# Twilight-Dream-Of-Magic/KolmogorovLike-DataCompressor

Measured on AMD Instinct MI355X. Metric: compress MB/s at fixed block size, bit-exact vs reference; 1/2/4/8-GPU scaling, higher is better.
Workload: dtype u8; 1 GPU; enwik-style synthetic text (kolm.datagen.enwik_like, seed 20251212+rank), 256 MiB per GPU resident in HBM, 1 MiB fixed blocks, candidates 0..8 + MDL, payloads emitted in HBM; block_size=1048576, bytes_per_gpu=268435456, blocks_per_gpu=256, parallelism=block-shard x1

## Files before the change

### kolmogorovlike-datacompressor_amd/csrc/k_mtf.hip

```cpp
#include "kolm_internal.h"

namespace kolm {

namespace {

struct ChunkGeom {
    Geom geo;
    u32 cpb;
    u32 csz;
    __device__ inline bool range(u32 c, u32& lo, u32& hi) const {
        const u32 b = c / cpb;
        const u32 k = c - b * cpb;
        lo = geo.base(b) + k * csz;
        const u32 e = geo.end(b);
        hi = min(lo + csz, e);
        return lo < e;
    }
};

constexpr u32 MTF_SLAB = 64;

__global__ __launch_bounds__(256) void k_mtf_summary(ChunkGeom cg, const u8* in, u8* summary,
                                                     u16* scnt, u32 nchunks) {
    __shared__ u32 sl[256 * MTF_SLAB / 4];
    __shared__ u32 slo[256];
    const u32 t = threadIdx.x;
    const u32 c = blockIdx.x * blockDim.x + t;
    u32 lo = 0, hi = 0;
    const bool valid = c < nchunks && cg.range(c, lo, hi);
    u16 cnt = 0;
    if (__syncthreads_and(valid && hi - lo == cg.csz && (lo & 15) == 0)) {
        u32 seen[8] = {0, 0, 0, 0, 0, 0, 0, 0};
        u8* out = summary + (u64)c * 256;
        slo[t] = lo;
        __syncthreads();
        for (u32 r = cg.csz; r > 0; r -= MTF_SLAB) {
#pragma unroll
            for (u32 q = 0; q < MTF_SLAB / 16; ++q) {
                const u32 m = q * 256 + t, owner = m >> 2, part = m & 3;
                reinterpret_cast<uint4*>(sl)[m] =
                    *reinterpret_cast<const uint4*>(in + slo[owner] + r - MTF_SLAB + 16 * part);
            }
            __syncthreads();
            const u32* slab = sl + t * (MTF_SLAB / 4);
#pragma unroll
            for (int q = MTF_SLAB / 4 - 1; q >= 0; --q) {
                const u32 wv = slab[q];
#pragma unroll
                for (int j = 3; j >= 0; --j) {
                    const u32 b = (wv >> (8 * j)) & 0xFF, w = b >> 5, bit = 1u << (b & 31);
                    u32 sw = 0;
#pragma unroll
                    for (int k = 0; k < 8; ++k) sw = (k == (int)w) ? seen[k] : sw;
                    if (!(sw & bit)) {
#pragma unroll
                        for (int k = 0; k < 8; ++k)
                            if (k == (int)w) seen[k] |= bit;
                        out[cnt++] = (u8)b;
                    }
                }
            }
            __syncthreads();
        }
        scnt[c] = cnt;
        return;
    }
    if (!valid) {
        if (c < nchunks) scnt[c] = 0;
        return;
    }
    {
        u32 seen[8] = {0, 0, 0, 0, 0, 0, 0, 0};
        u8* out = summary + (u64)c * 256;
        auto visit = [&](u32 b) {
            const u32 w = b >> 5, bit = 1u << (b & 31);
            u32 sw = 0;
#pragma unroll
            for (int k = 0; k < 8; ++k) sw = (k == (int)w) ? seen[k] : sw;
            if (!(sw & bit)) {
#pragma unroll
                for (int k = 0; k < 8; ++k)
                    if (k == (int)w) seen[k] |= bit;
                out[cnt++] = (u8)b;
            }
        };
        if (((lo | hi) & 15) == 0) {
            for (u32 i = hi; i > lo; i -= 16) {
                const uint4 v = *reinterpret_cast<const uint4*>(in + i - 16);
                const u32 wv[4] = {v.x, v.y, v.z, v.w};
#pragma unroll
                for (int q = 3; q >= 0; --q)
#pragma unroll
                    for (int j = 3; j >= 0; --j) visit((wv[q] >> (8 * j)) & 0xFF);
            }
        } else {
            for (u32 i = hi; i > lo; --i) visit(in[i - 1]);
        }
    }
    scnt[c] = cnt;
}

__device__ inline void mtf_apply(u32* st, u8* nst, u32* member, const u8* sm, u32 cnt) {
    const u32 lane = threadIdx.x & 63;
    if (lane < 8) member[lane] = 0;
    __builtin_amdgcn_wave_barrier();
    __builtin_amdgcn_fence(__ATOMIC_RELEASE, "wavefront");
    u32 sv[4];
#pragma unroll
    for (int j = 0; j < 4; ++j) {
        const u32 i = 4 * lane + j;
        sv[j] = i < cnt ? sm[i] : 0;
        if (i < cnt) atomicOr(&member[sv[j] >> 5], 1u << (sv[j] & 31));
    }
    __builtin_amdgcn_fence(__ATOMIC_ACQ_REL, "wavefront");
    __builtin_amdgcn_wave_barrier();
    const u32 word = st[lane];
    u32 keep = 0;
    u8 e[4];
#pragma unroll
    for (int j = 0; j < 4; ++j) {
        e[j] = (word >> (8 * j)) & 0xFF;
        const bool in_sum = (member[e[j] >> 5] >> (e[j] & 31)) & 1u;
        keep |= (in_sum ? 0u : 1u) << j;
    }
    const u32 nk = __popc(keep);
    u32 pos = cnt + wave_incl_scan(nk, OpAddU(), 0u) - nk;
#pragma unroll
    for (int j = 0; j < 4; ++j) {
        const u32 i = 4 * lane + j;
        if (i < cnt) nst[i] = (u8)sv[j];
        if ((keep >> j) & 1u) nst[pos++] = e[j];
    }
    __builtin_amdgcn_fence(__ATOMIC_ACQ_REL, "wavefront");
    __builtin_amdgcn_wave_barrier();
    st[lane] = reinterpret_cast<const u32*>(nst)[lane];
    __builtin_amdgcn_fence(__ATOMIC_ACQ_REL, "wavefront");
    __builtin_amdgcn_wave_barrier();
}


constexpr u32 CP_W = 16;
constexpr u32 CP_G = 8;
constexpr u32 CP_S = 16;
constexpr u32 CP_R = CP_G * CP_S;

__device__ inline u32 mtf_ident(u32 lane) {
    return (4 * lane) | ((4 * lane + 1) << 8) | ((4 * lane + 2) << 16) | ((4 * lane + 3) << 24);
}

__device__ inline void cp_range(const ChunkGeom& cg, u32 b, u32 r, u32& k0, u32& k1) {
    const u32 nch = (cg.geo.end(b) - cg.geo.base(b) + cg.csz - 1) / cg.csz;
    const u32 per = (nch + CP_R - 1) / CP_R;
    k0 = min(r * per, nch);
    k1 = min(k0 + per, nch);
}

__global__ __launch_bounds__(64 * CP_W) void k_mtf_cp1(ChunkGeom cg, const u8* summary, const u16* scnt, u32* rst,
                                                      u32* rdist) {
    __shared__ u32 st[CP_W][64];
    __shared__ u8 nst[CP_W][256];
    __shared__ u32 member[CP_W][8];
    __shared__ u32 uni[CP_W][8];
    const u32 lane = threadIdx.x & 63, w = threadIdx.x >> 6;
    const u32 gr = blockIdx.x * CP_W + w, b = gr / CP_R, r = gr - b * CP_R;
    if (b >= cg.geo.nb) return;
    u32 k0, k1;
    cp_range(cg, b, r, k0, k1);
    st[w][lane] = mtf_ident(lane);
    if (lane < 8) uni[w][lane] = 0;
    __builtin_amdgcn_wave_barrier();
    for (u32 k = k0; k < k1; ++k) {
        const u32 c = b * cg.cpb + k;
        const u8* sm = summary + (u64)c * 256;
        const u32 cnt = scnt[c];
#pragma unroll
        for (int j = 0; j < 4; ++j) {
            const u32 i = 4 * lane + j;
            if (i < cnt) atomicOr(&uni[w][sm[i] >> 5], 1u << (sm[i] & 31));
        }
        mtf_apply(st[w], nst[w], member[w], sm, cnt);
    }
    __builtin_amdgcn_fence(__ATOMIC_ACQ_REL, "wavefront");
    __builtin_amdgcn_wave_barrier();
    rst[(u64)gr * 64 + lane] = st[w][lane];
    if (lane == 0) {
        u32 d = 0;
        for (int q = 0; q < 8; ++q) d += __popc(uni[w][q]);
        rdist[gr] = d;
    }
}

__global__ __launch_bounds__(64 * CP_G) void k_mtf_cp2(const u32* rst, const u32* rdist, u32* rentry) {
    __shared__ u32 st[CP_G][64];
    __shared__ u8 nst[CP_G][256];
    __shared__ u32 member[CP_G][8];
    __shared__ u32 uni[CP_G][8];
    __shared__ u8 gsum[CP_G][256];
    __shared__ u32 gentry[CP_G][64];
    __shared__ u32 gdist[CP_G];
    const u32 lane = threadIdx.x & 63, g = threadIdx.x >> 6, b = blockIdx.x;
    const u64 r0 = (u64)b * CP_R + g * CP_S;
    st[g][lane] = mtf_ident(lane);
    if (lane < 8) uni[g][lane] = 0;
    __builtin_amdgcn_wave_barrier();
    for (u32 v = 0; v < CP_S; ++v) {
        const u8* sm = reinterpret_cast<const u8*>(rst + (r0 + v) * 64);
        const u32 cnt = rdist[r0 + v];
#pragma unroll
        for (int j = 0; j < 4; ++j) {
            const u32 i = 4 * lane + j;
            if (i < cnt) atomicOr(&uni[g][sm[i] >> 5], 1u << (sm[i] & 31));
        }
        mtf_apply(st[g], nst[g], member[g], sm, cnt);
    }
    __builtin_amdgcn_fence(__ATOMIC_ACQ_REL, "wavefront");
    __builtin_amdgcn_wave_barrier();
    reinterpret_cast<u32*>(gsum[g])[lane] = st[g][lane];
    if (lane == 0) {
        u32 d = 0;
        for (int q = 0; q < 8; ++q) d += __popc(uni[g][q]);
        gdist[g] = d;
    }
    __syncthreads();
    if (g == 0) {
        st[0][lane] = mtf_ident(lane);
        __builtin_amdgcn_wave_barrier();
        for (u32 v = 0; v < CP_G; ++v) {
            gentry[v][lane] = st[0][lane];
            __builtin_amdgcn_fence(__ATOMIC_ACQ_REL, "wavefront");
            __builtin_amdgcn_wave_barrier();
            if (v + 1 < CP_G) mtf_apply(st[0], nst[0], member[0], gsum[v], gdist[v]);
        }
    }
    __syncthreads();
    st[g][lane] = gentry[g][lane];
    __builtin_amdgcn_wave_barrier();
    for (u32 v = 0; v < CP_S; ++v) {
        rentry[(r0 + v) * 64 + lane] = st[g][lane];
        mtf_apply(st[g], nst[g], member[g], reinterpret_cast<const u8*>(rst + (r0 + v) * 64), rdist[r0 + v]);
    }
}

__global__ __launch_bounds__(64 * CP_W) void k_mtf_cp3(ChunkGeom cg, const u8* summary, const u16* scnt,
                                                      const u32* rentry, u8* states) {
    __shared__ u32 st[CP_W][64];
    __shared__ u8 nst[CP_W][256];
    __shared__ u32 member[CP_W][8];
    const u32 lane = threadIdx.x & 63, w = threadIdx.x >> 6;
    const u32 gr = blockIdx.x * CP_W + w, b = gr / CP_R, r = gr - b * CP_R;
    if (b >= cg.geo.nb) return;
    u32 k0, k1;
    cp_range(cg, b, r, k0, k1);
    st[w][lane] = rentry[(u64)gr * 64 + lane];
    __builtin_amdgcn_wave_barrier();
    for (u32 k = k0; k < k1; ++k) {
        const u32 c = b * cg.cpb + k;
        reinterpret_cast<u32*>(states + (u64)c * 256)[lane] = st[w][lane];
        mtf_apply(st[w], nst[w], member[w], summary + (u64)c * 256, scnt[c]);
    }
}

constexpr int RT = 128;

struct RiceAcc {
    u32 c[5] = {0, 0, 0, 0, 0};
    int k;
    u32 kk = 0, km = 0;
    __device__ inline void init(int rk) {
        k = rk;
        kk = rk < 8 ? (u32)rk : 0u;
        km = rk < 8 ? (0xFFu >> rk) * 0x01010101u : 0u;
    }
    __device__ inline u32 rb(u32 v) const { return (v >> k) + 1 + k; }
    __device__ inline u32 sum4(u32 w, u32 a) const { return __builtin_amdgcn_sad_u8((w >> kk) & km, 0u, a); }
    __device__ inline void add(u32 v) {
        c[0] += rb(v);
        c[2] += rb(((v & 0x0Fu) << 4) | (v >> 4));
        c[3] += rb(__brev(v) >> 24);
        c[4] += rb(v ^ (v >> 1));
    }
    __device__ inline void add4(u32 o) {
        const u32 one = 4 * (1 + k);
        c[0] = sum4(o, c[0] + one);
        c[2] = sum4(((o & 0x0F0F0F0Fu) << 4) | ((o >> 4) & 0x0F0F0F0Fu), c[2] + one);
        c[3] = sum4(__brev(o), c[3] + one);
        c[4] = sum4(o ^ ((o >> 1) & 0x7F7F7F7Fu), c[4] + one);
    }
    __device__ inline void group(u32 lo, u32 hi) {
        u64 x = ((u64)__builtin_bswap32(lo) << 32) | __builtin_bswap32(hi);
        u64 t = (x ^ (x >> 7)) & 0x00AA00AA00AA00AAull;
        x ^= t ^ (t << 7);
        t = (x ^ (x >> 14)) & 0x0000CCCC0000CCCCull;
        x ^= t ^ (t << 14);
        t = (x ^ (x >> 28)) & 0x00000000F0F0F0F0ull;
        x ^= t ^ (t << 28);
        c[1] = sum4((u32)(x >> 32), sum4((u32)x, c[1] + 8 * (1 + k)));
    }
};

__global__ __launch_bounds__(RT) void k_mtf_replay(ChunkGeom cg, const u8* in, const u8* states, u8* out,
                                                   u32 nchunks, u64* bits, int rice_k) {
    __shared__ u32 tab[64 * RT];
    const u32 t = threadIdx.x;
    const u32 c = blockIdx.x * RT + t;
    u32 lo = 0, hi = 0;
    const bool valid = c < nchunks && cg.range(c, lo, hi);
    u32 r0 = 0, r1 = 0;
    if (valid) {
        const u32* s = reinterpret_cast<const u32*>(states + (u64)c * 256);
        r0 = s[0];
        r1 = s[1];
        for (int w = 2; w < 64; ++w) tab[w * RT + t] = s[w];
    }
    auto haszero = [](u32 y) { return (y - 0x01010101u) & ~y & 0x80808080u; };
    auto front = [](u32 x, u32 j, u32 in) {
        const u32 lowmask = j ? ((1u << (8 * j)) - 1) : 0u;
        const u32 highmask = j == 3 ? 0u : ~((1u << (8 * (j + 1))) - 1);
        return (x & highmask) | ((x & lowmask) << 8) | in;
    };
    auto step = [&](u32 b) -> u32 {
        const u32 bb = b * 0x01010101u;
        u32 z = haszero(r0 ^ bb);
        if (z) {
            const u32 j = (__ffs(z) - 1) >> 3;
            r0 = front(r0, j, b);
            return j;
        }
        const u32 c0 = r0 >> 24;
        z = haszero(r1 ^ bb);
        if (z) {
            const u32 j = (__ffs(z) - 1) >> 3;
            r0 = (r0 << 8) | b;
            r1 = front(r1, j, c0);
            return 4 + j;
        }
        u32 w = 2, x;
        for (;;) {
            x = tab[w * RT + t];
            z = haszero(x ^ bb);
            if (z) break;
            ++w;
        }
        const u32 j = (__ffs(z) - 1) >> 3;
        u32 carry = r1 >> 24;
        r1 = (r1 << 8) | c0;
        r0 = (r0 << 8) | b;
        for (u32 v = 2; v < w; ++v) {
            const u32 xv = tab[v * RT + t];
            tab[v * RT + t] = (xv << 8) | carry;
            carry = xv >> 24;
        }
        tab[w * RT + t] = front(x, j, carry);
        return 4 * w + j;
    };
    RiceAcc acc;
    acc.init(rice_k);
    if (!valid) return;
    if (((lo | hi) & 63) == 0) {
        for (u32 i = lo; i < hi; i += 64) {
            uint4 v[4];
#pragma unroll
            for (int h = 0; h < 4; ++h) v[h] = *reinterpret_cast<const uint4*>(in + i + 16 * h);
            u32 ov[16];
#pragma unroll
            for (int q = 0; q < 16; ++q) {
                const u32 wq = q % 4 == 0 ? v[q / 4].x : q % 4 == 1 ? v[q / 4].y : q % 4 == 2 ? v[q / 4].z : v[q / 4].w;
                u32 o = 0;
#pragma unroll
                for (int j = 0; j < 4; ++j) o |= step((wq >> (8 * j)) & 0xFF) << (8 * j);
                ov[q] = o;
                if (bits) acc.add4(o);
                if (bits && (q & 1)) acc.group(ov[q - 1], o);
            }
#pragma unroll
            for (int h = 0; h < 4; ++h)
                *reinterpret_cast<uint4*>(out + i + 16 * h) = make_uint4(ov[4 * h], ov[4 * h + 1], ov[4 * h + 2], ov[4 * h + 3]);
        }
    } else if (((lo | hi) & 15) == 0) {
        for (u32 i = lo; i < hi; i += 16) {
            const uint4 v = *reinterpret_cast<const uint4*>(in + i);
            const u32 wv[4] = {v.x, v.y, v.z, v.w};
            u32 ov[4];
#pragma unroll
            for (int q = 0; q < 4; ++q) {
                u32 o = 0;
#pragma unroll
                for (int j = 0; j < 4; ++j) o |= step((wv[q] >> (8 * j)) & 0xFF) << (8 * j);
                ov[q] = o;
                if (bits) acc.add4(o);
            }
            *reinterpret_cast<uint4*>(out + i) = make_uint4(ov[0], ov[1], ov[2], ov[3]);
            if (bits) {
                acc.group(ov[0], ov[1]);
                acc.group(ov[2], ov[3]);
            }
        }
    } else {
        u32 g[2] = {0, 0}, gi = 0;
        for (u32 i = lo; i < hi; ++i) {
            const u32 m = step(in[i]);
            out[i] = (u8)m;
            if (bits) {
                acc.add(m);
                g[gi >> 2] |= m << (8 * (gi & 3));
                if (++gi == 8) {
                    acc.group(g[0], g[1]);
                    g[0] = g[1] = 0;
                    gi = 0;
                }
            }
        }
        if (bits && gi) acc.group(g[0], g[1]);
    }
    if (bits) {
        u64* dst = bits + (u64)(c / cg.cpb) * 8;
#pragma unroll
        for (int q = 0; q < 5; ++q)
            if (acc.c[q]) atomicAdd((unsigned long long*)&dst[q], (unsigned long long)acc.c[q]);
    }
}

__global__ __launch_bounds__(256) void k_mtf_wave(ChunkGeom cg, const u8* in, const u8* states, u8* out,
                                                  u32 nchunks, u64* bits, int rice_k) {
    __shared__ u32 st[4][64];
    __shared__ u8 nst[4][256];
    __shared__ u32 member[4][8];
    __shared__ u8 inv[4][256];
    __shared__ u8 smy[4][64];
    __shared__ __align__(8) u8 mb[4][64];
    const u32 w = threadIdx.x >> 6, lane = threadIdx.x & 63;
    const u32 c = blockIdx.x * 4 + w;
    u32 lo = 0, hi = 0;
    if (!(c < nchunks && cg.range(c, lo, hi))) return;
    {
        const u32 word = reinterpret_cast<const u32*>(states + (u64)c * 256)[lane];
        st[w][lane] = word;
#pragma unroll
        for (int j = 0; j < 4; ++j) inv[w][(word >> (8 * j)) & 0xFF] = (u8)(4 * lane + j);
    }
    __builtin_amdgcn_fence(__ATOMIC_ACQ_REL, "wavefront");
    __builtin_amdgcn_wave_barrier();
    RiceAcc acc;
    acc.init(rice_k);
    const u64 below = (1ull << lane) - 1ull;
    for (u32 p = lo; p < hi; p += 64) {
        const u32 i = p + lane;
        const bool v = i < hi;
        const u32 sym = v ? in[i] : 0u;
        const u64 vm = __ballot(v);
        const u32 mypos = inv[w][sym];
        u64 rem = vm, mine = 0;
        while (rem) {
            const u32 k = (u32)__ffsll((long long)rem) - 1;
            const u32 sk = __builtin_amdgcn_readlane(sym, k);
            const u64 eq = __ballot(v && sym == sk);
            if (sym == sk) mine = eq;
            rem &= ~eq;
        }
        const u64 pm = mine & below;
        const u32 prev = pm ? 63u - (u32)__clzll((long long)pm) : 0u;
        const u64 win = pm ? below & ~((2ull << prev) - 1ull) : 0ull;
        u32 cnt = 0, seen = 0, less = 0;
        rem = vm;
        while (rem) {
            const u32 k = (u32)__ffsll((long long)rem) - 1;
            const u32 sk = __builtin_amdgcn_readlane(sym, k);
            const u32 pk = __builtin_amdgcn_readlane(mypos, k);
            const u64 eq = __ballot(v && sym == sk);
            cnt += (eq & win) ? 1u : 0u;
            if (k < lane) {
                ++seen;
                less += pk < mypos ? 1u : 0u;
            }
            rem &= ~eq;
        }
        const u32 m = pm ? cnt : seen + mypos - less;
        if (v) out[i] = (u8)m;
        mb[w][lane] = v ? (u8)m : (u8)0;
        if (bits && v) acc.add(m);
        const bool last = v && (mine >> lane) == 1ull;
        const u64 lm = __ballot(last);
        if (last) smy[w][__popcll(lm >> lane) - 1] = (u8)sym;
        __builtin_amdgcn_fence(__ATOMIC_ACQ_REL, "wavefront");
        __builtin_amdgcn_wave_barrier();
        if (bits && (lane & 7) == 0 && v) {
            const u32* g = reinterpret_cast<const u32*>(&mb[w][lane]);
            acc.group(g[0], g[1]);
        }
        mtf_apply(st[w], nst[w], member[w], smy[w], (u32)__popcll(lm));
        const u32 word = st[w][lane];
#pragma unroll
        for (int j = 0; j < 4; ++j) inv[w][(word >> (8 * j)) & 0xFF] = (u8)(4 * lane + j);
        __builtin_amdgcn_fence(__ATOMIC_ACQ_REL, "wavefront");
        __builtin_amdgcn_wave_barrier();
    }
    if (bits) {
        u64* dst = bits + (u64)(c / cg.cpb) * 8;
#pragma unroll
        for (int q = 0; q < 5; ++q) {
            const u32 sum = wave_reduce(acc.c[q], OpAddU(), 0u);
            if (lane == 0 && sum) atomicAdd((unsigned long long*)&dst[q], (unsigned long long)sum);
        }
    }
}

}

bool mtf_wave_mode(const Geom& geo) {
    const char* e = getenv("KOLM_MTF_WAVE");
    const int force = e ? atoi(e) : -1;
    return force >= 0 ? force != 0 : geo.nb < 64;
}

u32 mtf_chunk_bytes(const Geom& geo) {
    static const u32 force = getenv("KOLM_MTF_CHUNK") ? (u32)atoi(getenv("KOLM_MTF_CHUNK")) : 0u;
    if (force >= 64 && force <= MTF_CHUNK && (force & (force - 1)) == 0) return force;
    u32 csz = MTF_CHUNK;
    if (mtf_wave_mode(geo)) return csz;
    while (csz > 128 && (u64)((geo.bs + csz - 1) / csz) * geo.nb < 16384) csz >>= 1;
    return csz;
}

u64 mtf_cp_words(const Geom& geo) { return (u64)geo.nb * CP_R * 129; }

void launch_mtf(const Geom& geo, const u8* in, u8* out, u8* summary, u16* summary_cnt, u8* states,
                hipStream_t s, KTimer* kt, u64* bits, int rice_k, u32* cp_scratch) {
    if (!geo.N) return;
    const u32 csz = mtf_chunk_bytes(geo);
    ChunkGeom cg{geo, (geo.bs + csz - 1) / csz, csz};
    const u32 nchunks = cg.cpb * geo.nb;
    const u64 N = geo.N;
    {
        KScope k(kt, KT_MTF, "k_mtf_summary", N + (u64)nchunks * 256);
        k_mtf_summary<<<(nchunks + 255) / 256, 256, 0, s>>>(cg, in, summary, summary_cnt, nchunks);
    }
    {
        KScope k(kt, KT_MTF, "k_mtf_compose", (u64)nchunks * 512);
        {
            u32* rst = cp_scratch;
            u32* rentry = cp_scratch + (u64)geo.nb * CP_R * 64;
            u32* rdist = rentry + (u64)geo.nb * CP_R * 64;
            const u32 g13 = (geo.nb * CP_R + CP_W - 1) / CP_W;
            k_mtf_cp1<<<g13, 64 * CP_W, 0, s>>>(cg, summary, summary_cnt, rst, rdist);
            k_mtf_cp2<<<geo.nb, 64 * CP_G, 0, s>>>(rst, rdist, rentry);
            k_mtf_cp3<<<g13, 64 * CP_W, 0, s>>>(cg, summary, summary_cnt, rentry, states);
        }
    }
    if (mtf_wave_mode(geo)) {
        KScope k(kt, KT_MTF, "k_mtf_wave", 2 * N + (u64)nchunks * 256);
        k_mtf_wave<<<(nchunks + 3) / 4, 256, 0, s>>>(cg, in, states, out, nchunks, bits, rice_k);
    } else {
        KScope k(kt, KT_MTF, "k_mtf_replay", 2 * N + (u64)nchunks * 256);
        k_mtf_replay<<<(nchunks + RT - 1) / RT, RT, 0, s>>>(cg, in, states, out, nchunks, bits, rice_k);
    }
}

}
```

Before: 8803 MB/s.

## Replace serial MTF range composition with last-occurrence key ranking

The per-range MTF state kernel previously applied each chunk summary sequentially with mtf_apply and atomic union bitmaps. It now records a last-seen key per symbol (chunk index and position stamp) in one pass over the summaries, four chunks at a time, then builds the final MTF order by ranking keys with a 64x4 comparison sweep. This replaces a long serial chain of wave-synchronised list updates with independent scatter writes plus one O(256^2) rank, and shrinks workgroups to 4 waves. It adds a 2^24-chunk limit check and relies on the key ordering reproducing MTF semantics exactly.

```diff
diff --git a/kolmogorovlike-datacompressor_amd/csrc/k_mtf.hip b/kolmogorovlike-datacompressor_amd/csrc/k_mtf.hip
--- a/kolmogorovlike-datacompressor_amd/csrc/k_mtf.hip
+++ b/kolmogorovlike-datacompressor_amd/csrc/k_mtf.hip
@@ -1,4 +1,5 @@
 #include "kolm_internal.h"
+#include "mtf_core.h"
 
 namespace kolm {
 
@@ -139,10 +140,13 @@
 }
 
 
-constexpr u32 CP_W = 16;
-constexpr u32 CP_G = 8;
-constexpr u32 CP_S = 16;
-constexpr u32 CP_R = CP_G * CP_S;
+constexpr u32 CP_W = 4;
+constexpr u32 RS_W = 4;
+constexpr u32 RS_B = 4;
+constexpr u32 CP_G = mtf::GROUPS;
+constexpr u32 CP_S = mtf::GROUP_RANGES;
+constexpr u32 CP_R = mtf::RANGES;
+static_assert(CP_R % RS_W == 0 && CP_R == CP_G * CP_S, "whole workgroups of ranges");
 
 __device__ inline u32 mtf_ident(u32 lane) {
     return (4 * lane) | ((4 * lane + 1) << 8) | ((4 * lane + 2) << 16) | ((4 * lane + 3) << 24);
@@ -150,44 +154,60 @@
 
 __device__ inline void cp_range(const ChunkGeom& cg, u32 b, u32 r, u32& k0, u32& k1) {
     const u32 nch = (cg.geo.end(b) - cg.geo.base(b) + cg.csz - 1) / cg.csz;
-    const u32 per = (nch + CP_R - 1) / CP_R;
-    k0 = min(r * per, nch);
-    k1 = min(k0 + per, nch);
-}
-
-__global__ __launch_bounds__(64 * CP_W) void k_mtf_cp1(ChunkGeom cg, const u8* summary, const u16* scnt, u32* rst,
-                                                      u32* rdist) {
-    __shared__ u32 st[CP_W][64];
-    __shared__ u8 nst[CP_W][256];
-    __shared__ u32 member[CP_W][8];
-    __shared__ u32 uni[CP_W][8];
-    const u32 lane = threadIdx.x & 63, w = threadIdx.x >> 6;
-    const u32 gr = blockIdx.x * CP_W + w, b = gr / CP_R, r = gr - b * CP_R;
+    mtf::range_chunks(nch, r, k0, k1);
+}
+
+__global__ __launch_bounds__(64 * RS_W) void k_mtf_rsum(ChunkGeom cg, const u8* __restrict__ summary,
+                                                        const u16* __restrict__ scnt, u32* __restrict__ rst,
+                                                        u32* __restrict__ rdist) {
+    __shared__ uint4 key[RS_W][64];
+    __shared__ __align__(4) u8 ost[RS_W][256];
+    const u32 lane = threadIdx.x & 63, w = __builtin_amdgcn_readfirstlane(threadIdx.x >> 6);
+    const u32 gr = blockIdx.x * RS_W + w, b = gr / CP_R, r = gr - b * CP_R;
     if (b >= cg.geo.nb) return;
     u32 k0, k1;
     cp_range(cg, b, r, k0, k1);
-    st[w][lane] = mtf_ident(lane);
-    if (lane < 8) uni[w][lane] = 0;
-    __builtin_amdgcn_wave_barrier();
-    for (u32 k = k0; k < k1; ++k) {
-        const u32 c = b * cg.cpb + k;
-        const u8* sm = summary + (u64)c * 256;
-        const u32 cnt = scnt[c];
-#pragma unroll
-        for (int j = 0; j < 4; ++j) {
-            const u32 i = 4 * lane + j;
-            if (i < cnt) atomicOr(&uni[w][sm[i] >> 5], 1u << (sm[i] & 31));
-        }
-        mtf_apply(st[w], nst[w], member[w], sm, cnt);
-    }
-    __builtin_amdgcn_fence(__ATOMIC_ACQ_REL, "wavefront");
-    __builtin_amdgcn_wave_barrier();
-    rst[(u64)gr * 64 + lane] = st[w][lane];
-    if (lane == 0) {
-        u32 d = 0;
-        for (int q = 0; q < 8; ++q) d += __popc(uni[w][q]);
-        rdist[gr] = d;
-    }
+    u32* kw = reinterpret_cast<u32*>(key[w]);
+    key[w][lane] = make_uint4(mtf::key_unseen(4 * lane), mtf::key_unseen(4 * lane + 1), mtf::key_unseen(4 * lane + 2),
+                              mtf::key_unseen(4 * lane + 3));
+    for (u32 k = k0; k < k1; k += RS_B) {
+        u32 cnt[RS_B], word[RS_B];
+#pragma unroll
+        for (u32 q = 0; q < RS_B; ++q) {
+            const u32 c = b * cg.cpb + min(k + q, k1 - 1);
+            cnt[q] = k + q < k1 ? (u32)scnt[c] : 0u;
+            word[q] = reinterpret_cast<const u32*>(summary + (u64)c * 256)[lane];
+        }
+#pragma unroll
+        for (u32 q = 0; q < RS_B; ++q)
+#pragma unroll
+            for (u32 j = 0; j < 4; ++j) {
+                const u32 i = 4 * lane + j;
+                if (i < cnt[q]) kw[(word[q] >> (8 * j)) & 0xFF] = mtf::key_seen(k + q - k0, i);
+            }
+    }
+    __builtin_amdgcn_fence(__ATOMIC_ACQ_REL, "wavefront");
+    __builtin_amdgcn_wave_barrier();
+    const uint4 mine = key[w][lane];
+    const u32 mk[4] = {mine.x, mine.y, mine.z, mine.w};
+    u32 rk[4] = {0, 0, 0, 0};
+#pragma unroll 8
+    for (u32 t = 0; t < 64; ++t) {
+        const uint4 o = key[w][t];
+#pragma unroll
+        for (u32 j = 0; j < 4; ++j)
+            rk[j] += mtf::above(o.x, mk[j]) + mtf::above(o.y, mk[j]) + mtf::above(o.z, mk[j]) + mtf::above(o.w, mk[j]);
+    }
+    u32 dist = 0;
+#pragma unroll
+    for (u32 j = 0; j < 4; ++j) {
+        ost[w][rk[j]] = (u8)(4 * lane + j);
+        dist += (u32)__popcll(__ballot(mtf::seen(mk[j])));
+    }
+    __builtin_amdgcn_fence(__ATOMIC_ACQ_REL, "wavefront");
+    __builtin_amdgcn_wave_barrier();
+    rst[(u64)gr * 64 + lane] = reinterpret_cast<const u32*>(ost[w])[lane];
+    if (lane == 0) rdist[gr] = dist;
 }
 
 __global__ __launch_bounds__(64 * CP_G) void k_mtf_cp2(const u32* rst, const u32* rdist, u32* rentry) {
@@ -530,6 +550,8 @@
     ChunkGeom cg{geo, (geo.bs + csz - 1) / csz, csz};
     const u32 nchunks = cg.cpb * geo.nb;
     const u64 N = geo.N;
+    if ((cg.cpb + CP_R - 1) / CP_R > mtf::PER_MAX)
+        throw HipError(hipErrorInvalidValue, "MTF: more than 2^24 chunks in a block", __LINE__);
     {
         KScope k(kt, KT_MTF, "k_mtf_summary", N + (u64)nchunks * 256);
         k_mtf_summary<<<(nchunks + 255) / 256, 256, 0, s>>>(cg, in, summary, summary_cnt, nchunks);
@@ -540,10 +562,9 @@
             u32* rst = cp_scratch;
             u32* rentry = cp_scratch + (u64)geo.nb * CP_R * 64;
             u32* rdist = rentry + (u64)geo.nb * CP_R * 64;
-            const u32 g13 = (geo.nb * CP_R + CP_W - 1) / CP_W;
-            k_mtf_cp1<<<g13, 64 * CP_W, 0, s>>>(cg, summary, summary_cnt, rst, rdist);
+            k_mtf_rsum<<<geo.nb * CP_R / RS_W, 64 * RS_W, 0, s>>>(cg, summary, summary_cnt, rst, rdist);
             k_mtf_cp2<<<geo.nb, 64 * CP_G, 0, s>>>(rst, rdist, rentry);
-            k_mtf_cp3<<<g13, 64 * CP_W, 0, s>>>(cg, summary, summary_cnt, rentry, states);
+            k_mtf_cp3<<<(geo.nb * CP_R + CP_W - 1) / CP_W, 64 * CP_W, 0, s>>>(cg, summary, summary_cnt, rentry, states);
         }
     }
     if (mtf_wave_mode(geo)) {
diff --git a/kolmogorovlike-datacompressor_amd/csrc/mtf_core.h b/kolmogorovlike-datacompressor_amd/csrc/mtf_core.h
--- /dev/null
+++ b/kolmogorovlike-datacompressor_amd/csrc/mtf_core.h
@@ -0,0 +1,37 @@
+#pragma once
+#include <cstdint>
+
+#if defined(__HIPCC__)
+#define MTF_HD __host__ __device__ inline
+#else
+#define MTF_HD inline
+#endif
+
+namespace mtf {
+
+typedef uint8_t u8;
+typedef uint16_t u16;
+typedef uint32_t u32;
+typedef uint64_t u64;
+
+constexpr u32 GROUPS = 8;
+constexpr u32 GROUP_RANGES = 16;
+constexpr u32 RANGES = GROUPS * GROUP_RANGES;
+constexpr u32 PER_MAX = (1u << 24) / RANGES;
+constexpr u32 KEY_SEEN = 256;
+static_assert(PER_MAX == 1u << 17, "2^24 chunks over 128 ranges");
+static_assert((u64{PER_MAX - 1} << 8) + 256 + 255 < (1u << 26), "a key is below 2^26");
+
+MTF_HD void range_chunks(u32 nch, u32 r, u32& k0, u32& k1) {
+    const u32 per = (nch + RANGES - 1) / RANGES;
+    k0 = r * per < nch ? r * per : nch;
+    k1 = k0 + per < nch ? k0 + per : nch;
+}
+
+MTF_HD u32 stamp(u32 j, u32 i) { return (j << 8) + (256 - i); }
+MTF_HD u32 key_seen(u32 j, u32 i) { return stamp(j, i) + 255; }
+MTF_HD u32 key_unseen(u32 s) { return 255 - s; }
+MTF_HD bool seen(u32 key) { return key >= KEY_SEEN; }
+MTF_HD u32 above(u32 kt, u32 ks) { return kt > ks ? 1u : 0u;  }
+
+}
```

Result: no change. 8772 MB/s (-0.4%).
